# EugenHotaj/pytorch-generative

Hardware: AMD Instinct MI355X
Metric: training images/sec (ImageGPT 8-block/4-head/16-embed, 28x28x1) (higher is better)
Workload: dtype f32; 1 GPU; BASELINE.json configs[1]: ImageGPT 8 blocks / 4 heads / 16 embed on 28x28x1 binarised-MNIST-shaped synthetic; one step = zero_grad + fwd + BCE + bwd + global grad-norm + Adam + lr decay (reference trainer.py:173-193); per_gpu_batch=1024, global_batch=1024, parallelism=dp1, launch=hipGraph replay

## Files before the change

### include/pg_hip.h

```cpp
#ifndef PG_HIP_H_
#define PG_HIP_H_

#include <stddef.h>
#include <stdint.h>

#ifdef __cplusplus
extern "C" {
#endif

#define PG_ABI_VERSION 1

#define PG_EINVAL (-1)
#define PG_ESHAPE (-2)

#define PG_MAX_TAPS 64

#define PG_ACT_NONE 0
#define PG_ACT_RELU 1
#define PG_ACT_ELU 2
#define PG_ACT_GELU 3
#define PG_ACT_ELU_OUT 4

#define PG_GATE_TANH 0
#define PG_GATE_IDENTITY 1
// ... 158 lines not shown
int pg_vec_mean_accum(const float* v, int n, float* out, void* stream);
int pg_fill_scaled(const float* g, float scale, float* out, int n, void* stream);

int pg_mlp_gelu_fwd(const float* x, const float* w1, const float* b1, const float* w2,
                    const float* b2, const float* res, float* y, int N, int C, int Hd, int L,
                    void* stream);
int pg_mlp_gelu_bwd(const float* x, const float* w1, const float* b1, const float* w2,
                    const float* dy, float* dx, float* dw1, float* db1, float* dw2, float* db2,
                    int N, int C, int Hd, int L, float* workspace, size_t workspace_floats,
                    void* stream);
size_t pg_mlp_gelu_bwd_workspace_floats(int N, int L);

int pg_gpt_block_head_fwd(const float* x, const float* ln_w, const float* ln_b, const float* wq,
                          const float* bq, const float* wkv, const float* bkv, float* qkv, int N,
                          int C, int L, float eps, void* stream);
int pg_gpt_block_head_bwd(const float* x, const float* ln_w, const float* ln_b, const float* wq,
                          const float* wkv, const float* dqkv, const float* gx, float* dx,
                          float* dln_w, float* dln_b, float* dwq, float* dbq, float* dwkv,
                          float* dbkv, int N, int C, int L, float eps, float* workspace,
                          size_t workspace_floats, void* stream);
size_t pg_gpt_block_head_bwd_workspace_floats(int N, int L);
int pg_gpt_block_tail_fwd(const float* o, const float* x, const float* wp, const float* bp,
                          const float* ln_w, const float* ln_b, const float* w1, const float* b1,
                          const float* w2, const float* b2, float* x_new, int N, int C, int Hd,
                          int L, float eps, void* stream);
int pg_gpt_block_tail_bwd(const float* o, const float* x, const float* wp, const float* bp,
                          const float* ln_w, const float* ln_b, const float* w1, const float* b1,
                          const float* w2, const float* dx_new, float* d_o, float* gx, float* dwp,
                          float* dbp, float* dln_w, float* dln_b, float* dw1, float* db1,
                          float* dw2, float* db2, int N, int C, int Hd, int L, float eps,
// ... 71 lines not shown
```

### pytorch-generative_amd/csrc/attention.hip

```cpp
#include <stdlib.h>

#include "attention_args.h"

namespace {

constexpr float NEG_BIG = -1.0e30f;
constexpr float POS_BIG = 1.0e30f;
constexpr int QPL = 2;

using AttnArgs = PgAttnArgs;

__device__ __forceinline__ float fast_exp2(float x) { return __builtin_amdgcn_exp2f(x); }

template <int DK, int DV> struct Cfg {
  static constexpr int RS = DK + DV;
  static constexpr int RS2 = DK + DV + 4;
  static constexpr int CH = (RS <= 8) ? 8 : ((RS <= 16) ? 4 : 2);
  static constexpr int CH2 = (CH > 2) ? CH / 2 : 2;
};

template <int DA, int DB, int RS>
__device__ __forceinline__ void stage_rows(float* __restrict__ tile, const float* __restrict__ a,
                                           int da, const float* __restrict__ b, int db, int L,
                                           int m0, int KT, int tid, int nthreads) {
// ... 487 lines not shown
PG_EXPORT int pg_causal_attn_fwd(const float* q, const float* k, const float* v, float* o,
                                 float* lse2, int N, int heads, int L, int dk, int dv, long q_bs,
                                 long k_bs, long v_bs, long o_bs, int strict, void* stream) {
  PG_REQUIRE(q && k && v && o && lse2, PG_EINVAL, "pg_causal_attn_fwd: null pointer");
  int rc = check_dims("pg_causal_attn_fwd", N, heads, L, dk, dv, strict);
  if (rc) return rc;
  AttnArgs a = {};
  a.q = q; a.k = k; a.v = v; a.o_out = o; a.lse2_out = lse2;
  a.N = N; a.heads = heads; a.L = L; a.dk_dim = dk; a.dv_dim = dv; a.strict = strict;
  a.q_bs = q_bs; a.k_bs = k_bs; a.v_bs = v_bs; a.o_bs = o_bs;
  a.scale = 1.f / sqrtf((float)dk);
  a.scale2 = a.scale * 1.44269504088896340736f;
  rc = launch_any(K_FWD, a, (hipStream_t)stream);
  PG_REQUIRE(rc == 0, rc, "pg_causal_attn_fwd: head dims (%d, %d) at L = %d are not instantiated: pad them to multiples of 16 and L to a multiple of 16 (ops.causal_attention does)", dk, dv, L);
  PG_LAUNCH_CHECK("pg_causal_attn_fwd");
  return 0;
}

namespace {
int attn_bwd_impl(int which_mask, const float* q, const float* k, const float* v, const float* o,
                  const float* d_o, const float* lse2, float* delta, float* dq, float* dk, float* dv,
                  int N, int heads, int L, int dk_dim, int dv_dim, long q_bs, long k_bs, long v_bs,
                  long o_bs, long do_bs, long dq_bs, long dk_bs, long dv_bs, int strict, void* stream) {
  PG_REQUIRE(q && k && v && o && d_o && lse2 && delta && dq && dk && dv, PG_EINVAL,
             "pg_causal_attn_bwd: null pointer");
  int rc = check_dims("pg_causal_attn_bwd", N, heads, L, dk_dim, dv_dim, strict);
  if (rc) return rc;
  AttnArgs a = {};
  a.q = q; a.k = k; a.v = v; a.o = o; a.d_o = d_o; a.lse2_in = lse2; a.delta = delta;
  a.dq = dq; a.dk = dk; a.dv = dv;
// ... 53 lines not shown
```

### pytorch-generative_amd/csrc/attention_args.h

```cpp
#pragma once
#include "common.h"

struct PgAttnArgs {
  const float* q; const float* k; const float* v; const float* o; const float* d_o;
  const float* lse2_in;
  float* o_out; float* lse2_out; float* delta; float* dq; float* dk; float* dv;
  int N, heads, L, dk_dim, dv_dim, strict;
  long q_bs, k_bs, v_bs, o_bs, do_bs, dq_bs, dk_bs, dv_bs;
  float scale, scale2;
  int blocks_per_wg;
  int kt, kt2;
  int lp, vec;
  unsigned char bcount[8];
  unsigned char blist[8][16];
};

enum { PG_ATTN_FWD = 0, PG_ATTN_DQ = 1, PG_ATTN_DKV = 2, PG_ATTN_BWD = 3  };

int pg_attn_mfma_launch(int which, const PgAttnArgs& a, hipStream_t st);
```

### pytorch-generative_amd/csrc/attention_mfma.hip

```cpp
#include <stdio.h>
#include <stdlib.h>

#include <type_traits>

#include "attention_args.h"

namespace {

typedef float f32x4 __attribute__((ext_vector_type(4)));
constexpr float NEG_BIG = -1.0e30f;
constexpr float POS_BIG = 1.0e30f;
constexpr float PSUM_TH = 1024.0f;

typedef __bf16 bf16x8 __attribute__((ext_vector_type(8)));
#define MFMA16(A, B, C) __builtin_amdgcn_mfma_f32_16x16x4f32((A), (B), (C), 0, 0, 0)
#define MFMA16B(A, B, C) __builtin_amdgcn_mfma_f32_16x16x32_bf16((A), (B), (C), 0, 0, 0)
#define MFMA4(A, B, C) __builtin_amdgcn_mfma_f32_4x4x1f32((A), (B), (C), 0, 0, 0)

__device__ __forceinline__ float ex2(float x) { return __builtin_amdgcn_exp2f(x); }

__device__ __forceinline__ void quad_all(float x, float (&out)[4]) {
  const int v = __float_as_int(x);
  out[0] = __int_as_float(__builtin_amdgcn_update_dpp(0, v, 0x00, 0xf, 0xf, true));
  out[1] = __int_as_float(__builtin_amdgcn_update_dpp(0, v, 0x55, 0xf, 0xf, true));
// ... 96 lines not shown

struct Ids {
  int wave, lane, qi, g, jc, qb4;
};
__device__ __forceinline__ Ids ids() {
  Ids d;
  d.wave = __builtin_amdgcn_readfirstlane(threadIdx.x >> 6);
  d.lane = threadIdx.x & 63;
  d.qi = d.lane & 15;
  d.g = d.lane >> 4;
  d.jc = d.lane & 3;
  d.qb4 = ((d.lane >> 2) & 3) * 4;
  return d;
}

__global__ void __launch_bounds__(512) attn_fwd_m44_kernel(const PgAttnArgs a) {
  extern __shared__ float4 lds4[];
  const int Lp = a.lp;
  bf16x8* kc0 = reinterpret_cast<bf16x8*>(lds4);
  bf16x8* kc2 = kc0 + Lp;
  float* vt = reinterpret_cast<float*>(kc2 + Lp);
  bf16x8* ones = reinterpret_cast<bf16x8*>(vt + 4 * Lp);
  const Ids d = ids();
  const int qi = d.qi, g = d.g, jc = d.jc;
  const int h = blockIdx.y, n = blockIdx.z;
  const int L = a.L;
  const int NB = (L + 63) >> 6;

  const float* qp = a.q + (size_t)n * a.q_bs + (size_t)h * 4 * L;
  const float* kp = a.k + (size_t)n * a.k_bs + (size_t)h * 4 * L;
  const float* vp = a.v + (size_t)n * a.v_bs + (size_t)h * 4 * L;
  float* op = a.o_out + (size_t)n * a.o_bs + (size_t)h * 4 * L;
  float* lsep = a.lse2_out + ((size_t)n * a.heads + h) * L;

  const int rows = 64 * NB;
  const int nmine = a.bcount[d.wave];
  for (int m0 = 0; m0 < rows; m0 += 2 * blockDim.x) {
    float kx[2][4], vx[2][4];
#pragma unroll
    for (int u = 0; u < 2; ++u) {
      const int m = m0 + u * blockDim.x + threadIdx.x;
      load_row4(kx[u], kp, L, m);
      load_row4(vx[u], vp, L, m);
    }
#pragma unroll
    for (int u = 0; u < 2; ++u) {
      const int m = m0 + u * blockDim.x + threadIdx.x;
      if (m < rows) {
        put_chunks(kc0, kc2, m, kx[u]);
#pragma unroll
        for (int dd = 0; dd < 4; ++dd) vt[dd * Lp + m] = vx[u][dd];
      }
    }
  }
  if (threadIdx.x == 0) *ones = ones_chunk();
  __syncthreads();
  if (nmine == 0) return;
  const bf16x8* abase = g == 3 ? ones : (g == 2 ? kc2 : kc0) + qi;
  const int astride = g == 3 ? 0 : 1;

  const f32x4 zero4 = {0.f, 0.f, 0.f, 0.f};
#pragma unroll 1
  for (int it = 0; it < nmine; ++it) {
    const int blk = a.blist[d.wave][it];
    const int q0 = 64 * blk;
    const int ngrp = min(4, (L - q0 + 15) >> 4);

    float mcur[4], lsum[4];
    bf16x8 bq[4];
    f32x4 acc[4];
    int qidx[4];
#pragma unroll
    for (int t = 0; t < 4; ++t) {
      qidx[t] = q0 + 16 * t + qi;
      float qv[4];
      load_row4(qv, qp, L, qidx[t]);
#pragma unroll
      for (int dd = 0; dd < 4; ++dd) qv[dd] *= a.scale2;
      mcur[t] = 0.f;
      bq[t] = resident_operand(qv, 0.f, g);
      lsum[t] = 0.f;
      acc[t] = zero4;
    }

    auto shift_max = [&](int t, float c) {
      const float alpha = ex2(-c);
      float al[4];
      quad_all(alpha, al);
      lsum[t] *= alpha;
#pragma unroll
      for (int i = 0; i < 4; ++i) acc[t][i] *= al[i];
// ... 615 lines not shown
static void attn_waves(int* w) {
  static const AttnWaveCfg cfg = []() {
    AttnWaveCfg c = {{4, 8, 4}};
    if (const char* e = PG_AB_ENV("PG_ATTN_WAVES")) {
      int f = 0, q = 0, k = 0;
      if (sscanf(e, "%d,%d,%d", &f, &q, &k) == 3 && f >= 1 && f <= 8 && q >= 1 && q <= 8 && k >= 1 && k <= 8)
        c = {{f, q, k}};
    }
    return c;
  }();
  w[0] = cfg.w[0]; w[1] = cfg.w[1]; w[2] = cfg.w[2];
}

int pg_attn_k4_launch(int which, const PgAttnArgs& a, hipStream_t st);

#include <atomic>
static std::atomic<int>& fused_bwd_flag() {
  static std::atomic<int> flag([]() { const char* e = PG_AB_ENV("PG_ATTN_FUSED_BWD"); return (e && e[0] == '0') ? 0 : 1; }());
  return flag;
}
static bool pg_attn_fused_bwd_enabled() { return fused_bwd_flag().load(std::memory_order_relaxed) != 0; }
PG_EXPORT int pg_attn_fused_bwd(int enable) {
  if (enable < 0) return fused_bwd_flag().load(std::memory_order_relaxed);
  return fused_bwd_flag().exchange(enable ? 1 : 0, std::memory_order_relaxed);
}

int pg_attn_mfma_launch(int which, const PgAttnArgs& a0, hipStream_t st) {
  if (which == PG_ATTN_BWD) {
    if (!pg_attn_fused_bwd_enabled()) return 0;
    if (a0.dk_dim != 4 || a0.dv_dim != 4) {
      static const bool k4_fused = []() { const char* e = PG_AB_ENV("PG_ATTN_FUSED_BWD_K4"); return !(e && e[0] == '0'); }();
      return k4_fused ? pg_attn_k4_launch(which, a0, st) : 0;
    }
  }
  if (a0.dk_dim != 4 || a0.dv_dim != 4) return pg_attn_k4_launch(which, a0, st);
  PgAttnArgs a = a0;
  const int NB = (a.L + 63) / 64;
  a.lp = 64 * NB + 16;
  static const bool dkv_bf16 = []() { const char* e = PG_AB_ENV("PG_ATTN_DKV_BF16"); return !(e && e[0] == '0'); }();
  const size_t planes = which == PG_ATTN_BWD ? 21
                        : which == PG_ATTN_DKV ? (dkv_bf16 ? 18 : 10) : (which == PG_ATTN_DQ ? 20 : 12);
  int wcfg[3];
  attn_waves(wcfg);
  static const int bwd_waves = []() {
    const char* e = PG_AB_ENV("PG_ATTN_BWD_WAVES");
    const int v = e ? atoi(e) : 8;
    return v >= 1 && v <= 8 ? v : 8;
  }();
  int W = which == PG_ATTN_BWD ? bwd_waves : wcfg[which];
  const size_t shmem = planes * (size_t)a.lp * sizeof(float) + (which == PG_ATTN_BWD ? 8 * 1024 : 16);
  if (shmem > 160 * 1024) return 0;
  if (which == PG_ATTN_DKV && dkv_bf16 && !PG_AB_ENV("PG_ATTN_WAVES")) W = 8;
  if (which == PG_ATTN_FWD && (long)a.N * a.heads <= 512 && !PG_AB_ENV("PG_ATTN_WAVES")) W = 8;
  if (W > NB) W = NB;
  if ((NB + W - 1) / W > 16) return 0;
  long load[8] = {0, 0, 0, 0, 0, 0, 0, 0};
  for (int w = 0; w < 8; ++w) a.bcount[w] = 0;
  for (int rank = NB - 1; rank >= 0; --rank) {
    const int blk = (which == PG_ATTN_DKV || which == PG_ATTN_BWD) ? NB - 1 - rank : rank;
    int best = 0;
    for (int w = 1; w < W; ++w)
      if (load[w] < load[best] && a.bcount[w] < 16) best = w;
    if (a.bcount[best] >= 16) return 0;
    a.blist[best][a.bcount[best]++] = (unsigned char)blk;
    load[best] += 4 * rank + 5;
  }
  a.vec = a.L % 4 == 0 ? 1 : 0;
  if (which == PG_ATTN_FWD)
    a.vec = a.vec && aligned16(a.o_out) && a.o_bs % 4 == 0;
  else if (which == PG_ATTN_DQ)
    a.vec = a.vec && aligned16(a.dq) && a.dq_bs % 4 == 0;
  else
    a.vec = a.vec && aligned16(a.dk) && aligned16(a.dv) && a.dk_bs % 4 == 0 && a.dv_bs % 4 == 0;
  dim3 grid(1u, (unsigned)a.heads, (unsigned)a.N);
  dim3 block((unsigned)(64 * W));
  const void* fn = which == PG_ATTN_FWD  ? reinterpret_cast<const void*>(attn_fwd_m44_kernel)
                   : which == PG_ATTN_BWD ? (a.lp == 848 ? reinterpret_cast<const void*>(attn_bwd_m44_kernel<848>)
                                             : a.lp == 1040 ? reinterpret_cast<const void*>(attn_bwd_m44_kernel<1040>)
                                                            : reinterpret_cast<const void*>(attn_bwd_m44_kernel<0>))
                   : which == PG_ATTN_DQ ? reinterpret_cast<const void*>(attn_dq_m44_kernel)
                   : dkv_bf16            ? reinterpret_cast<const void*>(attn_dkv_m44_kernel<true>)
                                         : reinterpret_cast<const void*>(attn_dkv_m44_kernel<false>);
  if (shmem > 64 * 1024) (void)hipFuncSetAttribute(fn, hipFuncAttributeMaxDynamicSharedMemorySize, (int)shmem);
  if (which == PG_ATTN_FWD)
    hipLaunchKernelGGL(attn_fwd_m44_kernel, grid, block, shmem, st, a);
  else if (which == PG_ATTN_BWD && a.lp == 848)
    hipLaunchKernelGGL(attn_bwd_m44_kernel<848>, grid, block, shmem, st, a);
  else if (which == PG_ATTN_BWD && a.lp == 1040)
    hipLaunchKernelGGL(attn_bwd_m44_kernel<1040>, grid, block, shmem, st, a);
  else if (which == PG_ATTN_BWD)
    hipLaunchKernelGGL(attn_bwd_m44_kernel<0>, grid, block, shmem, st, a);
  else if (which == PG_ATTN_DQ)
    hipLaunchKernelGGL(attn_dq_m44_kernel, grid, block, shmem, st, a);
  else if (dkv_bf16)
    hipLaunchKernelGGL(attn_dkv_m44_kernel<true>, grid, block, shmem, st, a);
  else
    hipLaunchKernelGGL(attn_dkv_m44_kernel<false>, grid, block, shmem, st, a);
  return 1;
}
```

### pytorch-generative_amd/pytorch_generative_amd/_lib.py

```python

import ctypes
import os

_HERE = os.path.dirname(os.path.abspath(__file__))
LIB_PATH = os.environ.get("PG_HIP_LIB") or os.path.join(_HERE, "lib", "libpg_hip.so")

ABI_VERSION = 1

c_f = ctypes.c_void_p
c_i = ctypes.c_int
c_l = ctypes.c_long
c_z = ctypes.c_size_t
c_s = ctypes.c_void_p
c_ip = ctypes.POINTER(ctypes.c_int)
c_flt = ctypes.c_float

SIGNATURES = {
    "pg_abi_version": (c_i, []),
    "pg_last_error": (ctypes.c_char_p, []),
    "pg_conv2d_taps": (
        c_i,
        [c_f, c_f, c_f, c_f, c_f, c_i, c_i, c_i, c_i, c_i, c_i, c_i, c_i, c_ip, c_ip, c_i, c_f, c_i,
         c_s],
    ),
# ... 17 lines not shown
    "pg_pack_conv_weight_frag2": (c_i, [c_f, c_f, c_f, c_i, c_i, c_i, c_i, c_i, c_ip, c_ip, c_i, c_i, c_s]),
    "pg_pack_conv_weight": (c_i, [c_f, c_f, c_i, c_i, c_i, c_i, c_i, c_ip, c_ip, c_i, c_i, c_s]),
    "pg_packed_weight_floats": (c_z, [c_i, c_i, c_i]),
    "pg_conv_b_pad": (c_i, [c_i]),
    "pg_conv2d_wgrad": (
        c_i,
        [c_f, c_f, c_f, c_f, c_i, c_i, c_i, c_i, c_i, c_i, c_i, c_i, c_i, c_i, c_ip, c_ip, c_ip,
         c_ip, c_i, c_f, c_z, c_s],
    ),
    "pg_conv2d_wgrad_workspace_floats": (c_z, [c_i, c_i, c_i]),
    "pg_mul_inplace": (c_i, [c_f, c_f, c_z, c_s]),
    "pg_nchw_layernorm_fwd": (c_i, [c_f, c_f, c_f, c_f, c_f, c_f, c_i, c_i, c_i, c_flt, c_s]),
    "pg_nchw_layernorm_bwd": (
        c_i, [c_f, c_f, c_f, c_f, c_f, c_f, c_f, c_f, c_i, c_i, c_i, c_f, c_z, c_s]),
    "pg_gpt_block_head_fwd": (c_i, [c_f] * 8 + [c_i, c_i, c_i, c_flt, c_s]),
    "pg_gpt_block_head_bwd": (c_i, [c_f] * 14 + [c_i, c_i, c_i, c_flt, c_f, c_z, c_s]),
    "pg_gpt_block_head_bwd_workspace_floats": (c_z, [c_i, c_i]),
    "pg_gpt_block_head_bwd_partial": (c_i, [c_f] * 8 + [c_i, c_i, c_i, c_flt, c_f, c_z, c_s]),
    "pg_gpt_blocks_reduce": (c_i, [c_i, ctypes.POINTER(ctypes.c_void_p), ctypes.POINTER(ctypes.c_void_p),
                                   ctypes.POINTER(ctypes.c_void_p), c_i, c_i, c_i, c_s]),
    "pg_gpt_block_tail_fwd": (c_i, [c_f] * 11 + [c_i, c_i, c_i, c_i, c_flt, c_s]),
    "pg_gpt_block_tail_bwd": (c_i, [c_f] * 20 + [c_i, c_i, c_i, c_i, c_flt, c_f, c_z, c_s]),
    "pg_gpt_block_tail_bwd_workspace_floats": (c_z, [c_i, c_i]),
    "pg_gpt_block_tail_bwd_partial": (c_i, [c_f] * 12 + [c_i, c_i, c_i, c_i, c_flt, c_f, c_z, c_s]),
    "pg_gpt_block_head_bwd_with_tail": (c_i, [c_f] * 14 + [c_i, c_i, c_i, c_flt, c_f, c_z] + [c_f] * 9 + [c_s]),
    "pg_sample_embed": (c_i, [c_f] * 5 + [c_i] * 10 + [c_f, c_s]),
    "pg_attn_decode": (c_i, [c_f] * 4 + [c_i] * 8 + [c_f, c_s]),
    "pg_mlp_gelu_fwd": (c_i, [c_f, c_f, c_f, c_f, c_f, c_f, c_f, c_i, c_i, c_i, c_i, c_s]),
    "pg_mlp_gelu_bwd": (
        c_i, [c_f, c_f, c_f, c_f, c_f, c_f, c_f, c_f, c_f, c_f, c_i, c_i, c_i, c_i, c_f, c_z, c_s]),
# ... 161 lines not shown
```

### pytorch-generative_amd/pytorch_generative_amd/models/autoregressive/image_gpt.py

```python

import os

import torch
from torch import nn

from pytorch_generative_amd import _lib
from pytorch_generative_amd import nn as pg_nn
from pytorch_generative_amd import ops
from pytorch_generative_amd.models import base

_BLOCK_CHAIN = os.environ.get("PG_BLOCK_CHAIN", "1") != "0"


class TransformerBlock(nn.Module):
    def __init__(self, n_channels, n_attention_heads):
        super().__init__()
        self._ln1 = pg_nn.NCHWLayerNorm(n_channels)
        self._ln2 = pg_nn.NCHWLayerNorm(n_channels)
        self._attn = pg_nn.CausalAttention(
            in_channels=n_channels,
            n_heads=n_attention_heads,
            embed_channels=n_channels,
            out_channels=n_channels,
        )
# ... 2 lines not shown
            nn.GELU(),
            pg_nn.Conv2d(in_channels=4 * n_channels, out_channels=n_channels, kernel_size=1),
        )

    def _fused_ok(self, x):
        return ops.gpt_block_supported(x, self._ln1, self._attn._q, self._attn._kv, self._attn._proj,
                                       self._ln2, self._out[0], self._out[2])

    def forward_plus_input(self, x, chain=None, flush=False):
        if not self._fused_ok(x):
            return ops.add(x, self.forward(x))
        attn = self._attn
        pair = {}
        if chain is not None:
            pair["chain"], pair["flush"] = chain, flush
        qkv, xs = ops.gpt_block_head(x, self._ln1, attn._q, attn._kv, pair)
        o = ops.causal_attention_qkv(qkv, attn._n_heads, attn._embed_channels, attn._out_channels,
                                     attn._mask_center)
        return ops.gpt_block_tail(o, xs, attn._proj, self._ln2, self._out[0], self._out[2], pair)

    def forward(self, x):
        y, x = self._ln1(x, skip=True)
        x = self._attn(y, res=x)
        y, x = self._ln2(x, skip=True)
        if ops.mlp_gelu_supported(y, self._out[0], self._out[2]):
            return ops.mlp_gelu(y, self._out[0], self._out[2], res=x)
        hidden = self._out[0](y)
        return self._out[2](hidden, in_act="gelu", res=x)


class ImageGPT(base.AutoregressiveModel):
    def __init__(
        self,
# ... 131 lines not shown
```

### pytorch-generative_amd/pytorch_generative_amd/ops/__init__.py

```python

from pytorch_generative_amd.ops._common import (
    ACT_NONE,
    ACT_RELU,
    ACT_ELU,
    ACT_GELU,
    ACT_ELU_OUT,
    GATE_TANH,
    GATE_IDENTITY,
    _ACT_IDS,
    _stream,
    RowDecode,
    _chk,
    _p,
    zeros,
    zeros_like,
    _sink,
    CONV_FMT_F32,
    CONV_FMT_B3,
    CONV_FMT_B3_GATE,
    FUSE_SKIP,
    _dense_per_image,
)
from pytorch_generative_amd.ops.elementwise import (
    _ConcatChannels,
# ... 39 lines not shown
    GradSlot,
    FUSE_DUAL,
    FUSE_GATE,
)
from pytorch_generative_amd.ops.gpt_block import (
    FUSE_MLP,
    mlp_gelu_supported,
    _MlpGelu,
    mlp_gelu,
    FUSE_BLOCK,
    DEFER_BLOCK_REDUCE,
    _grad_targets,
    new_block_chain,
    assert_no_pending_block_reductions,
    flush_block_reductions,
    _GPTBlockHead,
    _GPTBlockTail,
    gpt_block_supported,
    gpt_block_head,
    gpt_block_tail,
    _NCHWLayerNorm,
    nchw_layernorm,
    nchw_layernorm_skip,
)
from pytorch_generative_amd.ops.attention import (
    _CausalAttention,
    _CausalAttentionQKV,
    _MergeQKVWeight,
    merge_qkv_weight,
    set_deterministic,
    causal_attention_qkv,
    attention_dims_native,
    _pad16,
    causal_attention,
# ... 58 lines not shown
```

### pytorch-generative_amd/pytorch_generative_amd/ops/gpt_block.py

```python

import os

import torch

from pytorch_generative_amd import _lib
from pytorch_generative_amd.ops._common import _chk, _p, _sink, _stream, zeros, zeros_like


FUSE_MLP = os.environ.get("PG_FUSE_MLP", "1") != "0"


def mlp_gelu_supported(x, conv1, conv2):
    if not FUSE_MLP or conv1.bias is None or conv2.bias is None:
        return False
    w1, w2 = conv1.weight, conv2.weight
    return (tuple(w1.shape) == (64, 16, 1, 1) and tuple(w2.shape) == (16, 64, 1, 1)
            and x.shape[1] == 16 and (x.shape[2] * x.shape[3]) % 16 == 0)


class _MlpGelu(torch.autograd.Function):
    @staticmethod
    def forward(ctx, x, w1, b1, w2, b2, res, sinks):
        lib = _lib.load()
        x = _chk(x, "mlp_gelu.x")
# ... 89 lines not shown

def flush_block_reductions(chain, n, c, L):
    import ctypes

    lib = _lib.load()
    jobs = chain["jobs"]
    for i in range(0, len(jobs), 8):
        grp = jobs[i:i + 8]
        hw = (ctypes.c_void_p * len(grp))(*[j[0].data_ptr() for j in grp])
        tw = (ctypes.c_void_p * len(grp))(*[j[1].data_ptr() for j in grp])
        gr = (ctypes.c_void_p * (14 * len(grp)))(*[ptr for j in grp for ptr in j[2]])
        _lib.check(lib.pg_gpt_blocks_reduce(len(grp), hw, tw, gr, n, c, L, _stream()), "pg_gpt_blocks_reduce")
    jobs.clear()


class _GPTBlockHead(torch.autograd.Function):

    @staticmethod
    def forward(ctx, x, lnw, lnb, wq, bq, wkv, bkv, eps, params, pair=None):
        lib = _lib.load()
        ctx.pair = pair
        x_in = x
        x = _chk(x, "gpt_block_head.x")
        n, c, h, w = x.shape
        qkv = torch.empty((n, 3 * c, h, w), device=x.device, dtype=torch.float32)
        _lib.check(
            lib.pg_gpt_block_head_fwd(x.data_ptr(), lnw.data_ptr(), lnb.data_ptr(), wq.data_ptr(),
                                      bq.data_ptr(), wkv.data_ptr(), bkv.data_ptr(), qkv.data_ptr(),
                                      n, c, h * w, eps, _stream()),
            "pg_gpt_block_head_fwd",
        )
        ctx.save_for_backward(x, lnw, lnb, wq, wkv)
        ctx.eps, ctx.params = eps, params
        return qkv, x_in

    @staticmethod
    def backward(ctx, dqkv, gx):
        lib = _lib.load()
        x, lnw, lnb, wq, wkv = ctx.saved_tensors
        n, c, h, w = x.shape
        pending = ctx.pair.pop("tail", None) if ctx.pair is not None else None
        if dqkv is None:
            if pending is not None:
                raise RuntimeError("gpt_block_head: a deferred tail reduction is pending but the head has no gradient")
            return gx, None, None, None, None, None, None, None, None, None
        dqkv = _chk(dqkv, "gpt_block_head.dqkv")
        gx = zeros_like(x) if gx is None else _chk(gx, "gpt_block_head.gx")
        dx = torch.empty_like(x)
        tgt, ret = _grad_targets(ctx.params)
        ws_n = lib.pg_gpt_block_head_bwd_workspace_floats(n, h * w)
        ws = torch.empty(ws_n, device=x.device, dtype=torch.float32)
        head_args = (x.data_ptr(), lnw.data_ptr(), lnb.data_ptr(), wq.data_ptr(),
                     wkv.data_ptr(), dqkv.data_ptr(), gx.data_ptr(), dx.data_ptr(),
                     tgt[0].data_ptr(), tgt[1].data_ptr(), tgt[2].data_ptr(),
                     tgt[3].data_ptr(), tgt[4].data_ptr(), tgt[5].data_ptr(), n, c,
                     h * w, ctx.eps, ws.data_ptr(), ws_n)
        chain = ctx.pair.get("chain") if ctx.pair is not None else None
        if pending is not None and chain is not None and all(r is None for r in ret):
            t_ws, t = pending
            _lib.check(lib.pg_gpt_block_head_bwd_partial(*head_args[:8], *head_args[14:], _stream()),
                       "pg_gpt_block_head_bwd_partial")
            chain["jobs"].append((ws, t_ws, [g.data_ptr() for g in tgt] + [t[4].data_ptr(), t[5].data_ptr(), t[6].data_ptr(),
                                                                          t[7].data_ptr(), t[0].data_ptr(), t[1].data_ptr(),
                                                                          t[2].data_ptr(), t[3].data_ptr()], (tgt, t)))
            if ctx.pair.get("flush"):
                flush_block_reductions(chain, n, c, h * w)
            return (dx, *ret, None, None, None)
        if pending is not None:
            t_ws, t = pending
            _lib.check(
                lib.pg_gpt_block_head_bwd_with_tail(*head_args, t_ws.data_ptr(), t[4].data_ptr(), t[5].data_ptr(),
                                                    t[6].data_ptr(), t[7].data_ptr(), t[0].data_ptr(),
                                                    t[1].data_ptr(), t[2].data_ptr(), t[3].data_ptr(), _stream()),
                "pg_gpt_block_head_bwd_with_tail",
            )
        else:
            _lib.check(lib.pg_gpt_block_head_bwd(*head_args, _stream()), "pg_gpt_block_head_bwd")
        return (dx, *ret, None, None, None)


class _GPTBlockTail(torch.autograd.Function):

    @staticmethod
    def forward(ctx, o, x, wp, bp, lnw, lnb, w1, b1, w2, b2, eps, params, pair=None):
        lib = _lib.load()
        ctx.pair = pair
        o = _chk(o, "gpt_block_tail.o")
        x = _chk(x, "gpt_block_tail.x")
        n, c, h, w = x.shape
        x_new = torch.empty_like(x)
        _lib.check(
            lib.pg_gpt_block_tail_fwd(o.data_ptr(), x.data_ptr(), wp.data_ptr(), bp.data_ptr(),
                                      lnw.data_ptr(), lnb.data_ptr(), w1.data_ptr(), b1.data_ptr(),
# ... 41 lines not shown
def gpt_block_supported(x, ln1, q, kv, proj, ln2, fc1, fc2):
    if not FUSE_BLOCK or x.shape[1] != 16 or (x.shape[2] * x.shape[3]) % 16 != 0:
        return False
    shapes = (tuple(q.weight.shape), tuple(kv.weight.shape), tuple(proj.weight.shape),
              tuple(fc1.weight.shape), tuple(fc2.weight.shape))
    if shapes != ((16, 16, 1, 1), (32, 16, 1, 1), (16, 16, 1, 1), (64, 16, 1, 1), (16, 64, 1, 1)):
        return False
    if any(m.bias is None for m in (q, kv, proj, fc1, fc2)):
        return False
    return tuple(ln1.normalized_shape) == (16,) and tuple(ln2.normalized_shape) == (16,)


def gpt_block_head(x, ln1, q, kv, pair=None):
    params = (ln1.weight, ln1.bias, q.weight, q.bias, kv.weight, kv.bias)
    return _GPTBlockHead.apply(x, *params, float(ln1.eps), params, pair)


def gpt_block_tail(o, x, proj, ln2, fc1, fc2, pair=None):
    params = (proj.weight, proj.bias, ln2.weight, ln2.bias, fc1.weight, fc1.bias, fc2.weight, fc2.bias)
    return _GPTBlockTail.apply(o, x, *params, float(ln2.eps), params, pair)


class _NCHWLayerNorm(torch.autograd.Function):
    @staticmethod
    def forward(ctx, x, gamma, beta, eps, gg, gb, with_skip=False):
        lib = _lib.load()
        x_in = x
        x = _chk(x, "layernorm.x")
        n, c, h, w = x.shape
        if gamma.numel() != c:
# ... 60 lines not shown
```

Before: 100,800 images/s.

## Fuse LayerNorm and QKV projection into the MFMA attention forward kernel

```diff
diff --git a/include/pg_hip.h b/include/pg_hip.h
--- a/include/pg_hip.h
+++ b/include/pg_hip.h
@@ -196,6 +196,10 @@
 int pg_gpt_block_head_fwd(const float* x, const float* ln_w, const float* ln_b, const float* wq,
                           const float* bq, const float* wkv, const float* bkv, float* qkv, int N,
                           int C, int L, float eps, void* stream);
+int pg_gpt_block_head_attn_supported(int N, int C, int heads, int L);
+int pg_gpt_block_head_attn_fwd(const float* x, const float* ln_w, const float* ln_b, const float* wq,
+                               const float* bq, const float* wkv, const float* bkv, float* qkv, float* o,
+                               float* lse2, int N, int C, int heads, int L, float eps, int strict, void* stream);
 int pg_gpt_block_head_bwd(const float* x, const float* ln_w, const float* ln_b, const float* wq,
                           const float* wkv, const float* dqkv, const float* gx, float* dx,
                           float* dln_w, float* dln_b, float* dwq, float* dbq, float* dwkv,
diff --git a/pytorch-generative_amd/csrc/attention.hip b/pytorch-generative_amd/csrc/attention.hip
--- a/pytorch-generative_amd/csrc/attention.hip
+++ b/pytorch-generative_amd/csrc/attention.hip
@@ -525,6 +525,44 @@
   rc = launch_any(K_FWD, a, (hipStream_t)stream);
   PG_REQUIRE(rc == 0, rc, "pg_causal_attn_fwd: head dims (%d, %d) at L = %d are not instantiated: pad them to multiples of 16 and L to a multiple of 16 (ops.causal_attention does)", dk, dv, L);
   PG_LAUNCH_CHECK("pg_causal_attn_fwd");
+  return 0;
+}
+
+namespace {
+int head_attn_args(const char* who, AttnArgs& a, int N, int C, int heads, int L, int strict) {
+  int rc = check_dims(who, N, heads, L, 4, 4, strict);
+  if (rc) return rc;
+  a.N = N; a.heads = heads; a.L = L; a.strict = strict;
+  a.dk_dim = C / heads; a.dv_dim = C / heads;
+  a.q_bs = a.k_bs = a.v_bs = 3L * C * L; a.o_bs = (long)C * L;
+  a.scale = 1.f / sqrtf((float)a.dk_dim);
+  a.scale2 = a.scale * 1.44269504088896340736f;
+  return 0;
+}
+bool head_attn_shape_ok(int C, int heads) { return C == 16 && heads == 4; }
+}
+
+PG_EXPORT int pg_gpt_block_head_attn_supported(int N, int C, int heads, int L) {
+  if (N <= 0 || L <= 0 || N > 65535 || !head_attn_shape_ok(C, heads) || !use_mfma_attention()) return 0;
+  AttnArgs a = {};
+  if (head_attn_args("pg_gpt_block_head_attn_supported", a, N, C, heads, L, 0)) return 0;
+  return pg_attn_mfma_head_fwd(a, false, nullptr);
+}
+
+PG_EXPORT int pg_gpt_block_head_attn_fwd(const float* x, const float* ln_w, const float* ln_b, const float* wq,
+                                         const float* bq, const float* wkv, const float* bkv, float* qkv, float* o,
+                                         float* lse2, int N, int C, int heads, int L, float eps, int strict, void* stream) {
+  PG_REQUIRE(x && ln_w && ln_b && wq && bq && wkv && bkv && qkv && o && lse2, PG_EINVAL,
+             "pg_gpt_block_head_attn_fwd: null pointer");
+  PG_REQUIRE(C > 0 && heads > 0 && C % heads == 0, PG_EINVAL, "pg_gpt_block_head_attn_fwd: channels %d not divisible by heads %d", C, heads);
+  AttnArgs a = {};
+  int rc = head_attn_args("pg_gpt_block_head_attn_fwd", a, N, C, heads, L, strict);
+  if (rc) return rc;
+  a.x = x; a.ln_w = ln_w; a.ln_b = ln_b; a.wq = wq; a.bq = bq; a.wkv = wkv; a.bkv = bkv; a.qkv_out = qkv; a.eps = eps;
+  a.q = qkv; a.k = qkv + (size_t)C * L; a.v = qkv + (size_t)2 * C * L; a.o_out = o; a.lse2_out = lse2;
+  const bool took = head_attn_shape_ok(C, heads) && use_mfma_attention() && pg_attn_mfma_head_fwd(a, true, (hipStream_t)stream) == 1;
+  PG_REQUIRE(took, PG_ESHAPE, "pg_gpt_block_head_attn_fwd: not handled (C = %d, heads = %d, L = %d): run pg_gpt_block_head_fwd + pg_causal_attn_fwd", C, heads, L);
+  PG_LAUNCH_CHECK("pg_gpt_block_head_attn_fwd");
   return 0;
 }
 
diff --git a/pytorch-generative_amd/csrc/attention_args.h b/pytorch-generative_amd/csrc/attention_args.h
--- a/pytorch-generative_amd/csrc/attention_args.h
+++ b/pytorch-generative_amd/csrc/attention_args.h
@@ -13,8 +13,12 @@
   int lp, vec;
   unsigned char bcount[8];
   unsigned char blist[8][16];
+  const float* x; const float* ln_w; const float* ln_b; const float* wq; const float* bq; const float* wkv; const float* bkv;
+  float* qkv_out;
+  float eps;
 };
 
 enum { PG_ATTN_FWD = 0, PG_ATTN_DQ = 1, PG_ATTN_DKV = 2, PG_ATTN_BWD = 3  };
 
 int pg_attn_mfma_launch(int which, const PgAttnArgs& a, hipStream_t st);
+int pg_attn_mfma_head_fwd(const PgAttnArgs& a, bool launch, hipStream_t st);
diff --git a/pytorch-generative_amd/csrc/attention_mfma.hip b/pytorch-generative_amd/csrc/attention_mfma.hip
--- a/pytorch-generative_amd/csrc/attention_mfma.hip
+++ b/pytorch-generative_amd/csrc/attention_mfma.hip
@@ -134,6 +134,40 @@
   return d;
 }
 
+__device__ __forceinline__ void ln16_pixel(float (&v)[16], const float* g, const float* b, float eps) {
+  float s[4];
+#pragma unroll
+  for (int gg = 0; gg < 4; ++gg) s[gg] = (v[4 * gg] + v[4 * gg + 1]) + (v[4 * gg + 2] + v[4 * gg + 3]);
+  const float mu = ((s[0] + s[1]) + (s[2] + s[3])) * 0.0625f;
+#pragma unroll
+  for (int c = 0; c < 16; ++c) v[c] -= mu;
+#pragma unroll
+  for (int gg = 0; gg < 4; ++gg)
+    s[gg] = fmaf(v[4 * gg], v[4 * gg], fmaf(v[4 * gg + 1], v[4 * gg + 1], fmaf(v[4 * gg + 2], v[4 * gg + 2], v[4 * gg + 3] * v[4 * gg + 3])));
+  const float var = ((s[0] + s[1]) + (s[2] + s[3])) * 0.0625f + eps;
+  float rs = rsqrtf(var);
+  rs = rs * (1.5f - 0.5f * var * rs * rs);
+#pragma unroll
+  for (int c = 0; c < 16; ++c) v[c] = fmaf(v[c] * rs, g[c], b[c]);
+}
+__device__ __forceinline__ void proj4(float (&out)[4], const float* w, const float* bias, const float (&y)[16]) {
+#pragma unroll
+  for (int j = 0; j < 4; ++j) {
+    float acc = bias[j];
+#pragma unroll
+    for (int c = 0; c < 16; ++c) acc = fmaf(w[j * 16 + c], y[c], acc);
+    out[j] = acc;
+  }
+}
+__device__ __forceinline__ void load_row4_own(float (&x)[4], const float* src, int L, int m) {
+  const int mc = m < L ? m : L - 1;
+#pragma unroll
+  for (int dd = 0; dd < 4; ++dd) x[dd] = src[(size_t)dd * L + mc];
+#pragma unroll
+  for (int dd = 0; dd < 4; ++dd) x[dd] = m < L ? x[dd] : 0.f;
+}
+
+template <bool HEAD>
 __global__ void __launch_bounds__(512) attn_fwd_m44_kernel(const PgAttnArgs a) {
   extern __shared__ float4 lds4[];
   const int Lp = a.lp;
@@ -155,21 +189,67 @@
 
   const int rows = 64 * NB;
   const int nmine = a.bcount[d.wave];
-  for (int m0 = 0; m0 < rows; m0 += 2 * blockDim.x) {
-    float kx[2][4], vx[2][4];
-#pragma unroll
-    for (int u = 0; u < 2; ++u) {
-      const int m = m0 + u * blockDim.x + threadIdx.x;
-      load_row4(kx[u], kp, L, m);
-      load_row4(vx[u], vp, L, m);
-    }
-#pragma unroll
-    for (int u = 0; u < 2; ++u) {
-      const int m = m0 + u * blockDim.x + threadIdx.x;
-      if (m < rows) {
-        put_chunks(kc0, kc2, m, kx[u]);
-#pragma unroll
-        for (int dd = 0; dd < 4; ++dd) vt[dd * Lp + m] = vx[u][dd];
+  if constexpr (HEAD) {
+    const float* xp = a.x + (size_t)n * 16 * L;
+    float* qw = a.qkv_out + (size_t)n * 48 * L + (size_t)h * 4 * L;
+    const float* wq = a.wq + h * 64;
+    const float* wk = a.wkv + h * 64;
+    const float* wv = a.wkv + 256 + h * 64;
+    for (int m0 = 0; m0 < rows; m0 += 2 * blockDim.x) {
+      float xv[2][16];
+#pragma unroll
+      for (int u = 0; u < 2; ++u) {
+        const int m = m0 + u * blockDim.x + threadIdx.x;
+        const int mc = m < L ? m : L - 1;
+#pragma unroll
+        for (int c = 0; c < 16; ++c) xv[u][c] = xp[(size_t)c * L + mc];
+      }
+#pragma unroll
+      for (int u = 0; u < 2; ++u) {
+        const int m = m0 + u * blockDim.x + threadIdx.x;
+        if (m < rows) {
+          const bool ok = m < L;
+          float q4[4], k4[4], v4[4];
+          ln16_pixel(xv[u], a.ln_w, a.ln_b, a.eps);
+          proj4(q4, wq, a.bq + 4 * h, xv[u]);
+          proj4(k4, wk, a.bkv + 4 * h, xv[u]);
+          proj4(v4, wv, a.bkv + 16 + 4 * h, xv[u]);
+          if (ok) {
+#pragma unroll
+            for (int dd = 0; dd < 4; ++dd) {
+              qw[(size_t)dd * L + m] = q4[dd];
+              qw[(size_t)(16 + dd) * L + m] = k4[dd];
+              qw[(size_t)(32 + dd) * L + m] = v4[dd];
+            }
+          }
+#pragma unroll
+          for (int dd = 0; dd < 4; ++dd) {
+            k4[dd] = ok ? k4[dd] : 0.f;
+            v4[dd] = ok ? v4[dd] : 0.f;
+          }
+          put_chunks(kc0, kc2, m, k4);
+#pragma unroll
+          for (int dd = 0; dd < 4; ++dd) vt[dd * Lp + m] = v4[dd];
+        }
+      }
+    }
+  } else {
+    for (int m0 = 0; m0 < rows; m0 += 2 * blockDim.x) {
+      float kx[2][4], vx[2][4];
+#pragma unroll
+      for (int u = 0; u < 2; ++u) {
+        const int m = m0 + u * blockDim.x + threadIdx.x;
+        load_row4(kx[u], kp, L, m);
+        load_row4(vx[u], vp, L, m);
+      }
+#pragma unroll
+      for (int u = 0; u < 2; ++u) {
+        const int m = m0 + u * blockDim.x + threadIdx.x;
+        if (m < rows) {
+          put_chunks(kc0, kc2, m, kx[u]);
+#pragma unroll
+          for (int dd = 0; dd < 4; ++dd) vt[dd * Lp + m] = vx[u][dd];
+        }
       }
     }
   }
@@ -194,7 +274,8 @@
     for (int t = 0; t < 4; ++t) {
       qidx[t] = q0 + 16 * t + qi;
       float qv[4];
-      load_row4(qv, qp, L, qidx[t]);
+      if constexpr (HEAD) load_row4_own(qv, qp, L, qidx[t]);
+      else load_row4(qv, qp, L, qidx[t]);
 #pragma unroll
       for (int dd = 0; dd < 4; ++dd) qv[dd] *= a.scale2;
       mcur[t] = 0.f;
@@ -840,6 +921,11 @@
 
 int pg_attn_k4_launch(int which, const PgAttnArgs& a, hipStream_t st);
 
+static bool m44_dkv_bf16() {
+  static const bool on = []() { const char* e = PG_AB_ENV("PG_ATTN_DKV_BF16"); return !(e && e[0] == '0'); }();
+  return on;
+}
+
 #include <atomic>
 static std::atomic<int>& fused_bwd_flag() {
   static std::atomic<int> flag([]() { const char* e = PG_AB_ENV("PG_ATTN_FUSED_BWD"); return (e && e[0] == '0') ? 0 : 1; }());
@@ -851,19 +937,10 @@
   return fused_bwd_flag().exchange(enable ? 1 : 0, std::memory_order_relaxed);
 }
 
-int pg_attn_mfma_launch(int which, const PgAttnArgs& a0, hipStream_t st) {
-  if (which == PG_ATTN_BWD) {
-    if (!pg_attn_fused_bwd_enabled()) return 0;
-    if (a0.dk_dim != 4 || a0.dv_dim != 4) {
-      static const bool k4_fused = []() { const char* e = PG_AB_ENV("PG_ATTN_FUSED_BWD_K4"); return !(e && e[0] == '0'); }();
-      return k4_fused ? pg_attn_k4_launch(which, a0, st) : 0;
-    }
-  }
-  if (a0.dk_dim != 4 || a0.dv_dim != 4) return pg_attn_k4_launch(which, a0, st);
-  PgAttnArgs a = a0;
+static bool m44_plan(int which, PgAttnArgs& a, int& W, size_t& shmem) {
   const int NB = (a.L + 63) / 64;
   a.lp = 64 * NB + 16;
-  static const bool dkv_bf16 = []() { const char* e = PG_AB_ENV("PG_ATTN_DKV_BF16"); return !(e && e[0] == '0'); }();
+  const bool dkv_bf16 = m44_dkv_bf16();
   const size_t planes = which == PG_ATTN_BWD ? 21
                         : which == PG_ATTN_DKV ? (dkv_bf16 ? 18 : 10) : (which == PG_ATTN_DQ ? 20 : 12);
   int wcfg[3];
@@ -873,13 +950,13 @@
     const int v = e ? atoi(e) : 8;
     return v >= 1 && v <= 8 ? v : 8;
   }();
-  int W = which == PG_ATTN_BWD ? bwd_waves : wcfg[which];
-  const size_t shmem = planes * (size_t)a.lp * sizeof(float) + (which == PG_ATTN_BWD ? 8 * 1024 : 16);
-  if (shmem > 160 * 1024) return 0;
+  W = which == PG_ATTN_BWD ? bwd_waves : wcfg[which];
+  shmem = planes * (size_t)a.lp * sizeof(float) + (which == PG_ATTN_BWD ? 8 * 1024 : 16);
+  if (shmem > 160 * 1024) return false;
   if (which == PG_ATTN_DKV && dkv_bf16 && !PG_AB_ENV("PG_ATTN_WAVES")) W = 8;
   if (which == PG_ATTN_FWD && (long)a.N * a.heads <= 512 && !PG_AB_ENV("PG_ATTN_WAVES")) W = 8;
   if (W > NB) W = NB;
-  if ((NB + W - 1) / W > 16) return 0;
+  if ((NB + W - 1) / W > 16) return false;
   long load[8] = {0, 0, 0, 0, 0, 0, 0, 0};
   for (int w = 0; w < 8; ++w) a.bcount[w] = 0;
   for (int rank = NB - 1; rank >= 0; --rank) {
@@ -887,7 +964,7 @@
     int best = 0;
     for (int w = 1; w < W; ++w)
       if (load[w] < load[best] && a.bcount[w] < 16) best = w;
-    if (a.bcount[best] >= 16) return 0;
+    if (a.bcount[best] >= 16) return false;
     a.blist[best][a.bcount[best]++] = (unsigned char)blk;
     load[best] += 4 * rank + 5;
   }
@@ -898,9 +975,26 @@
     a.vec = a.vec && aligned16(a.dq) && a.dq_bs % 4 == 0;
   else
     a.vec = a.vec && aligned16(a.dk) && aligned16(a.dv) && a.dk_bs % 4 == 0 && a.dv_bs % 4 == 0;
+  return true;
+}
+
+int pg_attn_mfma_launch(int which, const PgAttnArgs& a0, hipStream_t st) {
+  if (which == PG_ATTN_BWD) {
+    if (!pg_attn_fused_bwd_enabled()) return 0;
+    if (a0.dk_dim != 4 || a0.dv_dim != 4) {
+      static const bool k4_fused = []() { const char* e = PG_AB_ENV("PG_ATTN_FUSED_BWD_K4"); return !(e && e[0] == '0'); }();
+      return k4_fused ? pg_attn_k4_launch(which, a0, st) : 0;
+    }
+  }
+  if (a0.dk_dim != 4 || a0.dv_dim != 4) return pg_attn_k4_launch(which, a0, st);
+  PgAttnArgs a = a0;
+  int W;
+  size_t shmem;
+  if (!m44_plan(which, a, W, shmem)) return 0;
+  const bool dkv_bf16 = m44_dkv_bf16();
   dim3 grid(1u, (unsigned)a.heads, (unsigned)a.N);
   dim3 block((unsigned)(64 * W));
-  const void* fn = which == PG_ATTN_FWD  ? reinterpret_cast<const void*>(attn_fwd_m44_kernel)
+  const void* fn = which == PG_ATTN_FWD  ? reinterpret_cast<const void*>(attn_fwd_m44_kernel<false>)
                    : which == PG_ATTN_BWD ? (a.lp == 848 ? reinterpret_cast<const void*>(attn_bwd_m44_kernel<848>)
                                              : a.lp == 1040 ? reinterpret_cast<const void*>(attn_bwd_m44_kernel<1040>)
                                                             : reinterpret_cast<const void*>(attn_bwd_m44_kernel<0>))
@@ -909,7 +1003,7 @@
                                          : reinterpret_cast<const void*>(attn_dkv_m44_kernel<false>);
   if (shmem > 64 * 1024) (void)hipFuncSetAttribute(fn, hipFuncAttributeMaxDynamicSharedMemorySize, (int)shmem);
   if (which == PG_ATTN_FWD)
-    hipLaunchKernelGGL(attn_fwd_m44_kernel, grid, block, shmem, st, a);
+    hipLaunchKernelGGL(attn_fwd_m44_kernel<false>, grid, block, shmem, st, a);
   else if (which == PG_ATTN_BWD && a.lp == 848)
     hipLaunchKernelGGL(attn_bwd_m44_kernel<848>, grid, block, shmem, st, a);
   else if (which == PG_ATTN_BWD && a.lp == 1040)
@@ -924,3 +1018,17 @@
     hipLaunchKernelGGL(attn_dkv_m44_kernel<false>, grid, block, shmem, st, a);
   return 1;
 }
+
+int pg_attn_mfma_head_fwd(const PgAttnArgs& a0, bool launch, hipStream_t st) {
+  static const bool fuse = []() { const char* e = PG_AB_ENV("PG_ATTN_FUSE_HEAD"); return !(e && e[0] == '0'); }();
+  if (!fuse || a0.heads != 4 || a0.dk_dim != 4 || a0.dv_dim != 4) return 0;
+  PgAttnArgs a = a0;
+  int W;
+  size_t shmem;
+  if (!m44_plan(PG_ATTN_FWD, a, W, shmem)) return 0;
+  if (!launch) return 1;
+  if (shmem > 64 * 1024)
+    (void)hipFuncSetAttribute(reinterpret_cast<const void*>(attn_fwd_m44_kernel<true>), hipFuncAttributeMaxDynamicSharedMemorySize, (int)shmem);
+  hipLaunchKernelGGL(attn_fwd_m44_kernel<true>, dim3(1u, (unsigned)a.heads, (unsigned)a.N), dim3((unsigned)(64 * W)), shmem, st, a);
+  return 1;
+}
diff --git a/pytorch-generative_amd/pytorch_generative_amd/_lib.py b/pytorch-generative_amd/pytorch_generative_amd/_lib.py
--- a/pytorch-generative_amd/pytorch_generative_amd/_lib.py
+++ b/pytorch-generative_amd/pytorch_generative_amd/_lib.py
@@ -55,6 +55,8 @@
     "pg_nchw_layernorm_bwd": (
         c_i, [c_f, c_f, c_f, c_f, c_f, c_f, c_f, c_f, c_i, c_i, c_i, c_f, c_z, c_s]),
     "pg_gpt_block_head_fwd": (c_i, [c_f] * 8 + [c_i, c_i, c_i, c_flt, c_s]),
+    "pg_gpt_block_head_attn_supported": (c_i, [c_i] * 4),
+    "pg_gpt_block_head_attn_fwd": (c_i, [c_f] * 10 + [c_i, c_i, c_i, c_i, c_flt, c_i, c_s]),
     "pg_gpt_block_head_bwd": (c_i, [c_f] * 14 + [c_i, c_i, c_i, c_flt, c_f, c_z, c_s]),
     "pg_gpt_block_head_bwd_workspace_floats": (c_z, [c_i, c_i]),
     "pg_gpt_block_head_bwd_partial": (c_i, [c_f] * 8 + [c_i, c_i, c_i, c_flt, c_f, c_z, c_s]),
diff --git a/pytorch-generative_amd/pytorch_generative_amd/models/autoregressive/image_gpt.py b/pytorch-generative_amd/pytorch_generative_amd/models/autoregressive/image_gpt.py
--- a/pytorch-generative_amd/pytorch_generative_amd/models/autoregressive/image_gpt.py
+++ b/pytorch-generative_amd/pytorch_generative_amd/models/autoregressive/image_gpt.py
@@ -40,9 +40,12 @@
         pair = {}
         if chain is not None:
             pair["chain"], pair["flush"] = chain, flush
-        qkv, xs = ops.gpt_block_head(x, self._ln1, attn._q, attn._kv, pair)
-        o = ops.causal_attention_qkv(qkv, attn._n_heads, attn._embed_channels, attn._out_channels,
-                                     attn._mask_center)
+        if ops.gpt_block_head_attention_supported(x, attn._n_heads):
+            o, xs = ops.gpt_block_head_attention(x, self._ln1, attn._q, attn._kv, attn._n_heads, attn._mask_center, pair)
+        else:
+            qkv, xs = ops.gpt_block_head(x, self._ln1, attn._q, attn._kv, pair)
+            o = ops.causal_attention_qkv(qkv, attn._n_heads, attn._embed_channels, attn._out_channels,
+                                         attn._mask_center)
         return ops.gpt_block_tail(o, xs, attn._proj, self._ln2, self._out[0], self._out[2], pair)
 
     def forward(self, x):
diff --git a/pytorch-generative_amd/pytorch_generative_amd/ops/__init__.py b/pytorch-generative_amd/pytorch_generative_amd/ops/__init__.py
--- a/pytorch-generative_amd/pytorch_generative_amd/ops/__init__.py
+++ b/pytorch-generative_amd/pytorch_generative_amd/ops/__init__.py
@@ -77,10 +77,14 @@
     new_block_chain,
     assert_no_pending_block_reductions,
     flush_block_reductions,
+    _head_backward,
     _GPTBlockHead,
+    _GPTBlockHeadAttention,
     _GPTBlockTail,
     gpt_block_supported,
     gpt_block_head,
+    gpt_block_head_attention_supported,
+    gpt_block_head_attention,
     gpt_block_tail,
     _NCHWLayerNorm,
     nchw_layernorm,
diff --git a/pytorch-generative_amd/pytorch_generative_amd/ops/gpt_block.py b/pytorch-generative_amd/pytorch_generative_amd/ops/gpt_block.py
--- a/pytorch-generative_amd/pytorch_generative_amd/ops/gpt_block.py
+++ b/pytorch-generative_amd/pytorch_generative_amd/ops/gpt_block.py
@@ -127,6 +127,44 @@
     jobs.clear()
 
 
+def _head_backward(pair, pending, params, eps, x, lnw, lnb, wq, wkv, dqkv, gx):
+    lib = _lib.load()
+    n, c, h, w = x.shape
+    dqkv = _chk(dqkv, "gpt_block_head.dqkv")
+    gx = zeros_like(x) if gx is None else _chk(gx, "gpt_block_head.gx")
+    dx = torch.empty_like(x)
+    tgt, ret = _grad_targets(params)
+    ws_n = lib.pg_gpt_block_head_bwd_workspace_floats(n, h * w)
+    ws = torch.empty(ws_n, device=x.device, dtype=torch.float32)
+    head_args = (x.data_ptr(), lnw.data_ptr(), lnb.data_ptr(), wq.data_ptr(),
+                 wkv.data_ptr(), dqkv.data_ptr(), gx.data_ptr(), dx.data_ptr(),
+                 tgt[0].data_ptr(), tgt[1].data_ptr(), tgt[2].data_ptr(),
+                 tgt[3].data_ptr(), tgt[4].data_ptr(), tgt[5].data_ptr(), n, c,
+                 h * w, eps, ws.data_ptr(), ws_n)
+    chain = pair.get("chain") if pair is not None else None
+    if pending is not None and chain is not None and all(r is None for r in ret):
+        t_ws, t = pending
+        _lib.check(lib.pg_gpt_block_head_bwd_partial(*head_args[:8], *head_args[14:], _stream()),
+                   "pg_gpt_block_head_bwd_partial")
+        chain["jobs"].append((ws, t_ws, [g.data_ptr() for g in tgt] + [t[4].data_ptr(), t[5].data_ptr(), t[6].data_ptr(),
+                                                                      t[7].data_ptr(), t[0].data_ptr(), t[1].data_ptr(),
+                                                                      t[2].data_ptr(), t[3].data_ptr()], (tgt, t)))
+        if pair.get("flush"):
+            flush_block_reductions(chain, n, c, h * w)
+        return dx, ret
+    if pending is not None:
+        t_ws, t = pending
+        _lib.check(
+            lib.pg_gpt_block_head_bwd_with_tail(*head_args, t_ws.data_ptr(), t[4].data_ptr(), t[5].data_ptr(),
+                                                t[6].data_ptr(), t[7].data_ptr(), t[0].data_ptr(),
+                                                t[1].data_ptr(), t[2].data_ptr(), t[3].data_ptr(), _stream()),
+            "pg_gpt_block_head_bwd_with_tail",
+        )
+    else:
+        _lib.check(lib.pg_gpt_block_head_bwd(*head_args, _stream()), "pg_gpt_block_head_bwd")
+    return dx, ret
+
+
 class _GPTBlockHead(torch.autograd.Function):
 
     @staticmethod
@@ -149,47 +187,66 @@
 
     @staticmethod
     def backward(ctx, dqkv, gx):
-        lib = _lib.load()
         x, lnw, lnb, wq, wkv = ctx.saved_tensors
-        n, c, h, w = x.shape
         pending = ctx.pair.pop("tail", None) if ctx.pair is not None else None
         if dqkv is None:
             if pending is not None:
                 raise RuntimeError("gpt_block_head: a deferred tail reduction is pending but the head has no gradient")
             return gx, None, None, None, None, None, None, None, None, None
-        dqkv = _chk(dqkv, "gpt_block_head.dqkv")
-        gx = zeros_like(x) if gx is None else _chk(gx, "gpt_block_head.gx")
-        dx = torch.empty_like(x)
-        tgt, ret = _grad_targets(ctx.params)
-        ws_n = lib.pg_gpt_block_head_bwd_workspace_floats(n, h * w)
-        ws = torch.empty(ws_n, device=x.device, dtype=torch.float32)
-        head_args = (x.data_ptr(), lnw.data_ptr(), lnb.data_ptr(), wq.data_ptr(),
-                     wkv.data_ptr(), dqkv.data_ptr(), gx.data_ptr(), dx.data_ptr(),
-                     tgt[0].data_ptr(), tgt[1].data_ptr(), tgt[2].data_ptr(),
-                     tgt[3].data_ptr(), tgt[4].data_ptr(), tgt[5].data_ptr(), n, c,
-                     h * w, ctx.eps, ws.data_ptr(), ws_n)
-        chain = ctx.pair.get("chain") if ctx.pair is not None else None
-        if pending is not None and chain is not None and all(r is None for r in ret):
-            t_ws, t = pending
-            _lib.check(lib.pg_gpt_block_head_bwd_partial(*head_args[:8], *head_args[14:], _stream()),
-                       "pg_gpt_block_head_bwd_partial")
-            chain["jobs"].append((ws, t_ws, [g.data_ptr() for g in tgt] + [t[4].data_ptr(), t[5].data_ptr(), t[6].data_ptr(),
-                                                                          t[7].data_ptr(), t[0].data_ptr(), t[1].data_ptr(),
-                                                                          t[2].data_ptr(), t[3].data_ptr()], (tgt, t)))
-            if ctx.pair.get("flush"):
-                flush_block_reductions(chain, n, c, h * w)
-            return (dx, *ret, None, None, None)
-        if pending is not None:
-            t_ws, t = pending
-            _lib.check(
-                lib.pg_gpt_block_head_bwd_with_tail(*head_args, t_ws.data_ptr(), t[4].data_ptr(), t[5].data_ptr(),
-                                                    t[6].data_ptr(), t[7].data_ptr(), t[0].data_ptr(),
-                                                    t[1].data_ptr(), t[2].data_ptr(), t[3].data_ptr(), _stream()),
-                "pg_gpt_block_head_bwd_with_tail",
-            )
-        else:
-            _lib.check(lib.pg_gpt_block_head_bwd(*head_args, _stream()), "pg_gpt_block_head_bwd")
+        dx, ret = _head_backward(ctx.pair, pending, ctx.params, ctx.eps, x, lnw, lnb, wq, wkv, dqkv, gx)
         return (dx, *ret, None, None, None)
+
+
+class _GPTBlockHeadAttention(torch.autograd.Function):
+
+    @staticmethod
+    def forward(ctx, x, lnw, lnb, wq, bq, wkv, bkv, eps, params, pair, n_heads, strict):
+        lib = _lib.load()
+        ctx.pair = pair
+        x_in = x
+        x = _chk(x, "gpt_block_head_attention.x")
+        n, c, h, w = x.shape
+        L = h * w
+        qkv = torch.empty((n, 3 * c, h, w), device=x.device, dtype=torch.float32)
+        o = torch.empty_like(x)
+        lse2 = torch.empty((n, n_heads, L), device=x.device, dtype=torch.float32)
+        _lib.check(
+            lib.pg_gpt_block_head_attn_fwd(x.data_ptr(), lnw.data_ptr(), lnb.data_ptr(), wq.data_ptr(), bq.data_ptr(),
+                                           wkv.data_ptr(), bkv.data_ptr(), qkv.data_ptr(), o.data_ptr(), lse2.data_ptr(),
+                                           n, c, n_heads, L, eps, int(strict), _stream()),
+            "pg_gpt_block_head_attn_fwd",
+        )
+        ctx.save_for_backward(x, lnw, lnb, wq, wkv, qkv, o, lse2)
+        ctx.eps, ctx.params, ctx.cfg = eps, params, (n_heads, int(strict))
+        return o, x_in
+
+    @staticmethod
+    def backward(ctx, d_o, gx):
+        lib = _lib.load()
+        x, lnw, lnb, wq, wkv, qkv, o, lse2 = ctx.saved_tensors
+        n_heads, strict = ctx.cfg
+        pending = ctx.pair.pop("tail", None) if ctx.pair is not None else None
+        if d_o is None:
+            if pending is not None:
+                raise RuntimeError("gpt_block_head_attention: a deferred tail reduction is pending but the head has no gradient")
+            return (gx,) + (None,) * 11
+        d_o = _chk(d_o, "gpt_block_head_attention.d_o")
+        n, c, h, w = x.shape
+        L = h * w
+        d = c // n_heads
+        dqkv = torch.empty_like(qkv)
+        delta = torch.empty_like(lse2)
+        base, gbase, bs = qkv.data_ptr(), dqkv.data_ptr(), 3 * c * L
+        _lib.check(
+            lib.pg_causal_attn_bwd(
+                base, base + 4 * c * L, base + 8 * c * L, o.data_ptr(), d_o.data_ptr(), lse2.data_ptr(), delta.data_ptr(),
+                gbase, gbase + 4 * c * L, gbase + 8 * c * L, n, n_heads, L, d, d, bs, bs, bs, c * L, c * L, bs, bs, bs,
+                strict, _stream(),
+            ),
+            "pg_causal_attn_bwd",
+        )
+        dx, ret = _head_backward(ctx.pair, pending, ctx.params, ctx.eps, x, lnw, lnb, wq, wkv, dqkv, gx)
+        return (dx, *ret, None, None, None, None, None)
 
 
 class _GPTBlockTail(torch.autograd.Function):
@@ -261,6 +318,16 @@
 def gpt_block_head(x, ln1, q, kv, pair=None):
     params = (ln1.weight, ln1.bias, q.weight, q.bias, kv.weight, kv.bias)
     return _GPTBlockHead.apply(x, *params, float(ln1.eps), params, pair)
+
+
+def gpt_block_head_attention_supported(x, n_heads):
+    n, c, h, w = x.shape
+    return bool(_lib.load().pg_gpt_block_head_attn_supported(n, c, int(n_heads), h * w))
+
+
+def gpt_block_head_attention(x, ln1, q, kv, n_heads, mask_center, pair=None):
+    params = (ln1.weight, ln1.bias, q.weight, q.bias, kv.weight, kv.bias)
+    return _GPTBlockHeadAttention.apply(x, *params, float(ln1.eps), params, pair, int(n_heads), bool(mask_center))
 
 
 def gpt_block_tail(o, x, proj, ln2, fc1, fc2, pair=None):
```

Measured after the change: 100,800 images/s (median of 5 runs). No clear change (+0.1%).
